# kcat/openal-soft

Measured on NVIDIA H100. Metric: voice-samples/s mixed (HRTF, bsinc24, 1024-frame updates), higher is better.
Workload: dtype f32

## Files before the change

### openal-soft_b200/csrc/mixer_kernels.cuh

```cuda
#pragma once
#include <cstdint>
#include <cuda_runtime.h>

#include "voice_structs.hpp"
#include "async_ptx.cuh"

namespace b200mix {

constexpr int kLine = 1024;
constexpr int kHrirLen = 128;
constexpr int kHist = 64;
constexpr int kEdge = 24;
constexpr int kPad = 48;
constexpr int kResBuf = kLine + 256 + kPad;
constexpr int kSrcSizeMax = kResBuf - kEdge;
constexpr int kAccumLen = kLine + kHrirLen;
constexpr float kSilence = 0.00001f;
constexpr float kEps = 1.1920929e-07f;

constexpr uint32_t kVfStatic = 1u<<2, kVfLooping = 1u<<3, kVfHrtf = 1u<<4;
constexpr uint32_t kVfFading = 1u<<8, kVfHaveBuffer = 1u<<9, kVfCoefDirty = 1u<<10;
constexpr uint32_t kUpNoBuffer = 1u<<11;
constexpr uint32_t kVfChannelMask = 0xffu<<16;

struct alignas(16) BufferRec {
    const void *data;
    uint32_t frames, type, channels, pad;
};

struct alignas(16) VoiceRec {
    uint32_t state;
    uint32_t flags;
    uint32_t buffer, resampler;
    int32_t  pos; uint32_t frac, step, loop_start;
    uint32_t loop_end; float bsinc_sf; uint32_t bsinc_m, bsinc_l;
    uint32_t bsinc_off, tgt_delay0, tgt_delay1; float tgt_gain;
    uint32_t old_delay0, old_delay1; float old_gain; uint32_t send_mask;
    uint32_t send_slot[kMaxSends]; uint32_t pad2[2];
    float prev[kPad];
    float hist[kHist];
};

struct VoiceResult { int32_t position; uint32_t position_frac, flags, buffers_done; };

struct alignas(16) FilterRec {
    float cur[2][5]; float tgt[2][5];
    float z[2][2];
    int32_t counter[2];
    uint32_t active;
    uint32_t pad[5];
};
static_assert(sizeof(FilterRec) == 128, "FilterRec layout");

struct MixParams {
    VoiceRec *voices; const BufferRec *buffers;
    float2 *hrtf_tgt; float2 *hrtf_old;
    float *dry_cur; float *dry_tgt;
    float *partial;
    VoiceResult *results;
    const float *bsinc_tab[3];
    const float *cubic_tab[2];
    uint32_t max_voices, frames, ir_pad, cd, num_sends;
    float *xscratch;
    uint32_t *sendinfo;
    const uint32_t *order;
    uint32_t num_order;
    FilterRec *filt;
    uint32_t filt_paths;
    const float *dline;
    uint4 *qhdr; const uint32_t *queue;
    uint32_t *claim;
};

constexpr uint32_t kMaxQueue = 32, kNoLoop = 0xffffffffu;

constexpr uint32_t kSiSend = 1u, kSiPlaying = 2u, kSiDeferred = 4u, kSiDirty = 8u, kSiDry = 16u,
    kSiHrtf = 32u;

__device__ __forceinline__ void group_sync(int id, int count)
{
    if(id == 1) asm volatile("bar.sync 1, %0;" :: "r"(count) : "memory");
    else asm volatile("bar.sync 2, %0;" :: "r"(count) : "memory");
}

__device__ __forceinline__ void prefetch_l2(const void *p)
{ asm volatile("prefetch.global.L2 [%0];" :: "l"(p)); }

__device__ __forceinline__ uint32_t sample_bytes(uint32_t type)
{ return type == 1u ? 2u : ((type == 0u || type >= 5u) ? 1u : (type == 4u ? 8u : 4u)); }

__device__ __forceinline__ void prefetch_span(const char *base, size_t bytes, size_t off,
    size_t len, int t, int gs)
{
    if(off >= bytes) return;
    if(off + len > bytes) len = bytes - off;
    const size_t first = off & ~size_t(127);
    for(size_t a = first + size_t(t)*128u;a < off + len;a += size_t(gs)*128u)
        prefetch_l2(base + a);
}

__device__ __forceinline__ float load_sample(const BufferRec &b, size_t idx)
{
    switch(b.type)
    {
    case 0: return (float(static_cast<const uint8_t*>(b.data)[idx]) - 128.0f) * (1.0f/128.0f);
    case 1: return float(static_cast<const int16_t*>(b.data)[idx]) * (1.0f/32768.0f);
    case 2: return float(static_cast<const int32_t*>(b.data)[idx]) * (1.0f/2147483648.0f);
    case 3: return static_cast<const float*>(b.data)[idx];
    case 4: return float(static_cast<const double*>(b.data)[idx]);
    }
    return 0.0f;
}

__device__ __forceinline__ void calc_buffer_size(uint32_t fracPos, uint32_t increment,
    uint32_t dstRemaining, uint32_t &dst, uint32_t &src)
{
    const uint32_t ext = increment <= 65536u;
    const uint64_t srcSize64 = ((uint64_t(dstRemaining - ext)*increment + fracPos) >> 16)
        + ext + kEdge;
    if(srcSize64 <= uint64_t(kSrcSizeMax)) { dst = dstRemaining; src = uint32_t(srcSize64); return; }
    const uint64_t dstSize64 = ((uint64_t(kSrcSizeMax - kEdge)<<16) - fracPos) / increment;
    if(dstSize64 < dstRemaining) { dst = uint32_t(dstSize64) & ~3u; src = kSrcSizeMax; return; }
    dst = dstRemaining; src = kSrcSizeMax;
}

__device__ __forceinline__ int32_t add_sat(int32_t a, int32_t b)
{
    long long r = (long long)a + b;
    r = r > 2147483647ll ? 2147483647ll : (r < -2147483648ll ? -2147483648ll : r);
    return int32_t(r);
}

__device__ __forceinline__ float to_float(uint8_t v) { return (float(v) - 128.0f) * (1.0f/128.0f); }
__device__ __forceinline__ float to_float(int16_t v) { return float(v) * (1.0f/32768.0f); }
__device__ __forceinline__ float to_float(int32_t v) { return float(v) * (1.0f/2147483648.0f); }
__device__ __forceinline__ float to_float(float v) { return v; }
__device__ __forceinline__ float to_float(double v) { return float(v); }
struct MulawByte { uint8_t v; };
struct AlawByte { uint8_t v; };
__device__ __forceinline__ float to_float(MulawByte b)
{
    const uint32_t u = (~uint32_t(b.v)) & 0xffu;
    const int s = int((((u & 0x0fu)<<3) + 0x84u) << ((u>>4)&7u)) - 0x84;
    return float((u & 0x80u) ? -s : s) * (1.0f/32768.0f);
}
__device__ __forceinline__ float to_float(AlawByte b)
{
    const uint32_t a = uint32_t(b.v) ^ 0x55u;
    const uint32_t e = (a>>4)&7u, m = a & 0x0fu;
    const int s = (e == 0u) ? int((m<<4) + 8u) : int(((m<<4) + 0x108u) << (e-1u));
    return float((a & 0x80u) ? s : -s) * (1.0f/32768.0f);
}

template<typename T> __device__ __forceinline__ T ld_raw(const T *p) { return __ldg(p); }
template<> __device__ __forceinline__ MulawByte ld_raw(const MulawByte *p)
{ return MulawByte{__ldg(reinterpret_cast<const uint8_t*>(p))}; }
template<> __device__ __forceinline__ AlawByte ld_raw(const AlawByte *p)
{ return AlawByte{__ldg(reinterpret_cast<const uint8_t*>(p))}; }

constexpr int kPackB = 688;
static_assert(kPackB >= (kResBuf + 8 + 1)/2 && kPackB + (kResBuf + 8 + 1)/2 <= kResBuf + 8 + 24
    && (kPackB % 32) == 16, "16-bit window copies must fit the float window's storage");

__device__ __forceinline__ float win_at(const float *win, bool packed, uint32_t k)
{
    if(!packed) return win[k];
    const uint16_t y = reinterpret_cast<const uint16_t*>(win)[k];
    return float(int(y) - 32768) * (1.0f/32768.0f);
}

struct FillArgs {
    float *dst; uint32_t count, uintPos, q0, firstRun, loopStart, loopSize, lastFrame, channels;
    bool looping, pastEnd, simpleWrap;
};

__device__ __forceinline__ void filter_clear(FilterRec &fr, int t)
{
    if(t < 10) fr.cur[t/5][t%5] = fr.tgt[t/5][t%5];
    else if(t < 14) fr.z[(t-10)>>1][(t-10)&1] = 0.0f;
    else if(t < 16) fr.counter[t-14] = 0;
}

template<typename T, int GS>
__device__ __forceinline__ void fill_window(const FillArgs &A, const T *__restrict__ src, int t)
{
    for(uint32_t k0 = t;k0 < A.count;k0 += 8u*GS)
    {
        T raw[8];
        #pragma unroll
        for(int u = 0;u < 8;++u)
        {
            uint32_t k = k0 + uint32_t(u)*GS;
            k = k < A.count ? k : A.count-1u;
            uint32_t q;
            if(!A.looping) q = min(A.uintPos + k, A.lastFrame);
            else if(k < A.firstRun) q = A.q0 + k;
            else if(A.simpleWrap) q = A.loopStart + (k - A.firstRun);
            else q = A.loopStart + (k - A.firstRun)%A.loopSize;
            raw[u] = ld_raw(src + size_t(q)*A.channels);
        }
        #pragma unroll
        for(int u = 0;u < 8;++u)
        {
            const uint32_t k = k0 + uint32_t(u)*GS;
            if(k < A.count) A.dst[k] = A.pastEnd ? 0.0f : to_float(raw[u]);
        }
    }
}

constexpr int kWinFloats = kResBuf + 8 + 24;
template<int CDR>
struct alignas(16) GroupSmem {
    static constexpr int kTabStride = kPad + 2;
    float win[kWinFloats];
    alignas(8) float tabF[32*kTabStride];
    alignas(8) float tabD[32*kTabStride];
    float x[CDR > 0 ? kLine : 1];
    float newGain[32];
    uint64_t tmaBar;
    uint32_t claimed;
};

template<int GS, int OPT, int FP>
struct alignas(16) FirSmem {
    static constexpr int kLLen = FP + OPT*GS;
    static constexpr int kOLen = FP + kHist + FP + 32;
    float2 lLR[kLLen];
    float2 oLR[kOLen];
    float x[kHist + kLine];
    float2 coefT[kHrirLen], coefO[kHrirLen];
};

__device__ __forceinline__ float2 fma2_rn(float2 a, float2 b, float2 c)
{ return make_float2(__fmaf_rn(a.x, b.x, c.x), __fmaf_rn(a.y, b.y, c.y)); }

template<int OPT, int FP>
__device__ __forceinline__ void fir_pass(float2 (&acc)[OPT], const float2 *__restrict__ in,
    const float2 *__restrict__ coef, int irpad, int t0)
{
    constexpr int JB = 8;
    constexpr int W = OPT + JB - 1;
    for(int jb = 0;jb < irpad;jb += 2*JB)
    {
        const float2 *p = in + FP + t0 - jb - (JB-1);
        float2 w[W];
        #pragma unroll
        for(int k = 0;k < W;++k) w[k] = p[k];
        #pragma unroll
        for(int jj = 0;jj < JB;++jj)
        {
            const float2 c = coef[jb+jj];
            #pragma unroll
            for(int r = 0;r < OPT;++r)
                acc[r] = fma2_rn(c, w[r - jj + (JB-1)], acc[r]);
        }
        if(jb + JB >= irpad) break;
        #pragma unroll
        for(int k = W-1;k >= JB;--k) w[k] = w[k-JB];
        #pragma unroll
        for(int k = 0;k < JB;++k) w[k] = p[k - JB];
        #pragma unroll
        for(int jj = 0;jj < JB;++jj)
        {
            const float2 c = coef[jb+JB+jj];
            #pragma unroll
            for(int r = 0;r < OPT;++r)
                acc[r] = fma2_rn(c, w[r - jj + (JB-1)], acc[r]);
        }
    }
}

__device__ __forceinline__ uint32_t claim_voice(const MixParams &P, uint32_t &slot, int t, int bar,
    int gs, uint32_t groups)
{
    group_sync(bar, gs);
    if(t == 0)
    {
        uint32_t oi = atomicAdd(P.claim, 1u);
        if(oi >= P.num_order && atomicAdd(P.claim + 1, 1u) == groups - 1u)
        {
            atomicExch(P.claim, 0u);
            atomicExch(P.claim + 1, 0u);
        }
        slot = oi;
    }
    group_sync(bar, gs);
    return slot;
}


__device__ __forceinline__ bool voice_early_out(const MixParams &P, VoiceRec &rec, uint32_t v,
    uint32_t vstate, uint4 h1, int t)
{
    if(vstate != 1u && vstate != 2u)
    {
        if(t == 0)
        {
            if(P.results) P.results[v] = VoiceResult{int32_t(h1.x), h1.y, 1u<<7, 0u};
            if(P.sendinfo) P.sendinfo[v] = 0u;
        }
        return true;
    }
    if(h1.z < 1u)
    {
        if(t == 0)
        {
            if(vstate == 2u) rec.state = 0u;
            if(P.sendinfo) P.sendinfo[v] = 0u;
            if(P.results)
                P.results[v] = VoiceResult{int32_t(h1.x), h1.y, (vstate == 2u) ? (1u<<7) : 1u, 0u};
        }
        return true;
    }
    return false;
}

template<int GS>
__device__ __forceinline__ void build_phase_table(const MixParams &P, float *tabF, float *tabD,
    uint32_t resampler, uint32_t increment, uint4 h2, uint4 h3, int t,
    uint32_t &m, uint32_t &tapOff, uint32_t &ms)
{
    m = 0; tapOff = 0; ms = 5;
    if(resampler >= 4u)
    {
        m = h2.z;
        tapOff = kEdge - h2.w;
        const float *tab = P.bsinc_tab[(resampler-4u)>>1] + h3.x;
        const bool full = (increment > 65536u) && (resampler & 1u);
        const float sf = __uint_as_float(h2.y);
        const uint32_t rowLen = 2u*m;
        const float *tab2 = tab + 64u*m;
        ms = m + 1u;
        for(uint32_t c = t;c < rowLen;c += GS)
        {
            float *dstc = (c < m) ? (tabF + c) : (tabD + (c - m));
            #pragma unroll 1
            for(uint32_t p0 = 0;p0 < 32u;p0 += 8u)
            {
                float a[8], b[8];
                #pragma unroll
                for(int u = 0;u < 8;++u)
                {
                    a[u] = __ldg(tab + (p0+u)*rowLen + c);
                    b[u] = full ? __ldg(tab2 + (p0+u)*rowLen + c) : 0.0f;
                }
                #pragma unroll
                for(int u = 0;u < 8;++u)
                    dstc[(p0+u)*ms] = full ? fmaf(sf, b[u], a[u]) : a[u];
            }
        }
    }
    else if(resampler >= 2u)
    {
        m = 4; tapOff = kEdge - 1; ms = 5;
        const float *tab = P.cubic_tab[resampler-2u];
        for(uint32_t e = t;e < 128u;e += GS)
        {
            const uint32_t pi = e>>2, j = e&3u;
            tabF[pi*ms + j] = tab[pi*8u + j];
            tabD[pi*ms + j] = tab[pi*8u + 4u + j];
        }
    }
}

template<int GS>
__device__ __forceinline__ void prefetch_next_voices(const MixParams &P, uint32_t oi, uint32_t groups,
    int t)
{
    const uint32_t o2 = oi + 2u*groups, o1 = oi + groups;
    const uint32_t v2 = o2 < P.num_order ? P.order[o2] : 0xffffffffu;
    const uint32_t v1 = o1 < P.num_order ? P.order[o1] : 0xffffffffu;
    if(v2 < P.max_voices && t < 5)
        prefetch_l2(reinterpret_cast<const char*>(&P.voices[v2]) + t*128);
    if(v1 < P.max_voices)
    {
        const VoiceRec &nx = P.voices[v1];
        if((nx.state == 1u || nx.state == 2u) && (nx.flags & kVfHaveBuffer) && nx.step >= 1u)
        {
            const BufferRec nb = P.buffers[nx.buffer];
            const size_t fb = size_t(sample_bytes(nb.type))*nb.channels;
            const size_t bytes = size_t(nb.frames)*fb;
            const uint32_t p0 = nx.pos < 0 ? 0u : uint32_t(nx.pos);
            const size_t need = size_t((uint64_t(P.frames)*nx.step + nx.frac) >> 16) + kPad;
            const char *base = static_cast<const char*>(nb.data);
            prefetch_span(base, bytes, size_t(p0)*fb, need*fb, t, GS);
            if((nx.flags & kVfLooping) && p0 + need > nx.loop_end && nx.loop_end > p0)
                prefetch_span(base, bytes, size_t(nx.loop_start)*fb,
                    (p0 + need - nx.loop_end)*fb, t, GS);
        }
    }
}

template<int GS>
__device__ __forceinline__ void hold_end_sample(float *srcBuffer, uint32_t srcn, int t, int bar)
{
    const uint32_t avail = srcn < uint32_t(kEdge) ? srcn : uint32_t(kEdge);
    const uint32_t tofill = srcn > uint32_t(kEdge) ? srcn : uint32_t(kEdge);
    uint32_t best = 0;
    for(uint32_t i = 1;i < avail;++i)
        if(fabsf(srcBuffer[i]) < fabsf(srcBuffer[best])) best = i;
    const float held = srcBuffer[best];
    group_sync(bar, GS);
    for(uint32_t k = best+1+t;k < tofill;k += GS) srcBuffer[k] = held;
}

template<int GS>
__device__ __forceinline__ void pack_span16(float *win, const unsigned char *raw, uint32_t lead,
    uint32_t srcDelay, uint32_t count, int t, int bar)
{
    constexpr int NW = (kResBuf + 8 + 1)/2;
    constexpr int PER = (NW + GS - 1)/GS;
    static_assert((GS/32)*(32*PER - 1) >= NW + 1, "the warps' runs must cover every word");
    const uint32_t lane = uint32_t(t) & 31u;
    const uint32_t w0 = uint32_t(t >> 5)*(32u*PER - 1u) + lane;
    const uint32_t lo = uint32_t(kEdge) + srcDelay;
    const uint32_t nw = (min(lo + count + 8u, uint32_t(kResBuf + 8)) + 1u)/2u;
    const uint32_t off = lo - lead;
    const uint32_t *rw = reinterpret_cast<const uint32_t*>(raw) - int((off + 1u) >> 1);
    const uint32_t sh = (off & 1u)*16u;
    uint32_t wa[PER];
    #pragma unroll
    for(int u = 0;u < PER;++u)
    {
        const uint32_t w = w0 + uint32_t(u)*32u;
        wa[u] = (w <= nw && 2u*w + 1u >= lo) ? rw[w] : 0u;
    }
    #pragma unroll
    for(int u = 0;u < PER;++u)
    {
        const uint32_t w = w0 + uint32_t(u)*32u;
        uint32_t r1 = __shfl_sync(0xffffffffu, (u + 1 < PER && lane == 0u) ? wa[u + 1 < PER ? u + 1 : u] : wa[u],
            (lane + 1u) & 31u);
        if(u + 1 == PER && lane == 31u && w <= nw && 2u*w + 3u >= lo) r1 = rw[w + 1u];
        uint32_t a = __funnelshift_r(wa[u], r1, sh) ^ 0x80008000u;
        const int d = int(lo) - int(2u*w);
        const uint32_t m = (d >= 1 ? 0x0000ffffu : 0u) | (d >= 2 ? 0xffff0000u : 0u);
        a = (a & ~m) | (0x80008000u & m);
        if(u == 0 && w < uint32_t(kEdge/2))
            a = uint32_t(uint16_t(__float2int_rn(win[2u*w]*32768.0f) + 32768))
                | (uint32_t(uint16_t(__float2int_rn(win[2u*w + 1u]*32768.0f) + 32768)) << 16);
        wa[u] = a;
    }
    group_sync(bar, GS);
    uint32_t *pa = reinterpret_cast<uint32_t*>(win);
    uint32_t *pb = pa + kPackB;
    #pragma unroll
    for(int u = 0;u < PER;++u)
    {
        const uint32_t w = w0 + uint32_t(u)*32u;
        const uint32_t next = __shfl_sync(0xffffffffu, (u + 1 < PER && lane == 0u) ? wa[u + 1 < PER ? u + 1 : u] : wa[u],
            (lane + 1u) & 31u);
        if(w < nw)
        {
            if(u > 0 || lane > 0u || t < 32) pa[w] = wa[u];
            if(u + 1 < PER || lane < 31u) pb[w] = __funnelshift_r(wa[u], next, 16u);
        }
    }
}

template<int GS>
__device__ __forceinline__ bool stage_span_tma(float *win, uint64_t *tmaBar, uint32_t &tmaPhase,
    const BufferRec &buf, uint32_t flags, bool isQueue, bool looping, uint32_t loopStart,
    uint32_t loopEnd, uint32_t uintPos, uint32_t srcDelay, uint32_t count, bool pack, bool &packed,
    int t, int bar)
{
    if(isQueue || buf.type != 1u || buf.channels != 1u || ((flags >> 16) & 0xffu) != 0u || count == 0u)
        return false;
    const uint32_t loopSize = looping ? (loopEnd - loopStart) : 1u;
    const uint32_t q0 = !looping ? uintPos : ((uintPos < loopEnd) ? uintPos
        : ((uintPos-loopStart)%loopSize + loopStart));
    const uint32_t run1 = looping ? min(count, loopEnd - q0) : count;
    const uint32_t run2 = count - run1;
    const bool fits = looping ? (run2 <= loopSize && loopEnd <= buf.frames)
                              : (uintPos + count <= buf.frames);
    if(!fits) return false;
    const int16_t *base = static_cast<const int16_t*>(buf.data);
    const uintptr_t a1 = reinterpret_cast<uintptr_t>(base + q0);
    const uintptr_t a2 = reinterpret_cast<uintptr_t>(base + loopStart);
    const uint32_t lead1 = uint32_t(a1 & 15u) >> 1, lead2 = uint32_t(a2 & 15u) >> 1;
    const uint32_t bytes1 = ((run1 + lead1)*2u + 15u) & ~15u;
    const uint32_t bytes2 = run2 ? (((run2 + lead2)*2u + 15u) & ~15u) : 0u;
    constexpr uint32_t kWinBytes = uint32_t(kWinFloats*sizeof(float));
    unsigned char *wbytes = reinterpret_cast<unsigned char*>(win);
    unsigned char *raw2 = wbytes + kWinBytes - bytes2;
    unsigned char *raw1 = raw2 - bytes1;
    if(t == 0)
    {
        fence_proxy_async_smem();
        mbar_expect_tx(tmaBar, bytes1 + bytes2);
        bulk_g2s(raw1, reinterpret_cast<const void*>(a1 & ~uintptr_t(15)), bytes1, tmaBar);
        if(run2)
            bulk_g2s(raw2, reinterpret_cast<const void*>(a2 & ~uintptr_t(15)), bytes2, tmaBar);
    }
    mbar_wait(tmaBar, tmaPhase);
    tmaPhase ^= 1u;
    if(pack && !run2)
    {
        pack_span16<GS>(win, raw1, lead1, srcDelay, count, t, bar);
        packed = true;
        return true;
    }
    float *dst = win + kEdge + srcDelay;
    const int16_t *r1 = reinterpret_cast<const int16_t*>(raw1) + lead1;
    const int16_t *r2 = reinterpret_cast<const int16_t*>(raw2) + lead2;
    constexpr int PERW = (kSrcSizeMax + GS - 1)/GS;
    float v[PERW];
    #pragma unroll
    for(int u = 0;u < PERW;++u)
    {
        const uint32_t k = uint32_t(t) + uint32_t(u)*GS;
        int16_t x = 0;
        if(k < count) x = k < run1 ? r1[k] : r2[k - run1];
        v[u] = to_float(x);
    }
    group_sync(bar, GS);
    #pragma unroll
    for(int u = 0;u < PERW;++u)
    {
        const uint32_t k = uint32_t(t) + uint32_t(u)*GS;
        if(k < count) dst[k] = v[u];
    }
    return true;
}

template<int GS>
__device__ __forceinline__ bool gather_span(const MixParams &P, const BufferRec &buf, uint32_t flags,
    bool isQueue, uint4 qh, const uint32_t *qitems, bool looping, uint32_t loopStart, uint32_t loopEnd,
    uint32_t uintPos, uint32_t count, float *dst, int t, int bar)
{
    uint32_t done = 0, item = qh.x ? qh.y : kNoLoop, qpos = uintPos;
    bool more = true, winInt = true;
    while(more)
    {
// ... 252 lines not shown
    {
        const float cg = counter ? cur[c] : tgt[c];
        const float tg = playing ? tgt[c] : 0.0f;
        const float step = (tg - cg)*delta;
        const bool fade = fabsf(step) > kEps;
        const bool early = fade && fadeLen < counter;
        const float flat = (!early && fabsf(tg) > kSilence) ? tg : 0.0f;
        const uint32_t start = fade ? fadeLen : 0u;
        #pragma unroll
        for(int r = 0;r < SPT;++r)
        {
            const uint32_t i = t + r*GS;
            float gsel = 0.0f;
            if(i < n)
                gsel = (fade && i < fadeLen) ? (cg + step*float(i)) : (i >= start ? flat : 0.0f);
            const float x = xs[i < n ? i : 0];
            if(c < uint32_t(CDR))
            {
                #pragma unroll
                for(int cc = 0;cc < CDR;++cc)
                    if(cc == int(c)) accD[cc][r] = __fmaf_rn(x, gsel, accD[cc][r]);
            }
        }
        if(t == 0)
            newGain[c] = early ? (cg + step*float(fadeLen)) : tg;
    }
}

__device__ __forceinline__ void store_dry_gains(float *cur, const float *newGain, uint32_t cd, int t)
{
    if(t == 0)
        for(uint32_t c = 0;c < cd;++c) cur[c] = newGain[c];
}

__device__ __forceinline__ void write_back_voice(const MixParams &P, VoiceRec &rec, uint32_t v,
    uint4 h1, uint32_t flags, uint32_t vstate, uint32_t increment, bool haveBuffer, bool isQueue,
    uint4 qh, const uint32_t *qitems, bool looping, uint32_t loopStart, uint32_t loopEnd,
    uint32_t bufFrames)
{
    uint32_t newFlags = (flags | kVfFading) & ~kVfCoefDirty;
    uint32_t newState = vstate;
    uint32_t buffersDone = 0u;
    int32_t pos = int32_t(h1.x); uint32_t frac = h1.y;
    if(vstate == 2u) newState = 0u;
    else
    {
        frac += increment*P.frames;
        const uint32_t done = frac >> 16;
        pos = add_sat(pos, int32_t(done));
        frac &= 0xffffu;
        if(haveBuffer && pos > 0 && isQueue)
        {
            uint32_t item = qh.x ? qh.y : kNoLoop;
            while(item != kNoLoop)
            {
                const uint32_t len = P.buffers[qitems[item]].frames;
                if(len > uint32_t(pos)) break;
                pos -= int32_t(len);
                ++buffersDone;
                item = (item + 1u < qh.x) ? item + 1u : qh.z;
            }
            if(item == kNoLoop) { newFlags &= ~kVfHaveBuffer; newState = 2u; }
            else if(item != qh.y) P.qhdr[v].y = item;
        }
        else if(haveBuffer && pos > 0)
        {
            if(looping)
            {
                uint32_t up = uint32_t(pos);
                if(up >= loopEnd)
                    pos = int32_t((up-loopStart)%(loopEnd-loopStart) + loopStart);
            }
            else if(uint32_t(pos) >= bufFrames)
            {
                newFlags &= ~kVfHaveBuffer;
                newState = 2u;
            }
        }
        rec.pos = pos; rec.frac = frac;
    }
    rec.flags = newFlags;
    rec.state = newState;
    if(P.results)
        P.results[v] = VoiceResult{pos, frac,
            newState == 1u ? 1u : (newState == 2u ? 2u : (1u<<7)), buffersDone};
}

template<int GS, int GROUPS, int CDR>
__device__ __forceinline__ void store_partial_row(const float (&accD)[CDR][kLine/GS], unsigned char *smem,
    float *partial, int g, int t)
{
    constexpr int SPT = kLine / GS;
    const size_t row = blockIdx.x;
    __syncthreads();
    float *stage = reinterpret_cast<float*>(smem);
    float *pd = partial + row*(size_t(CDR)*kLine);
    if(GROUPS == 1)
    {
        #pragma unroll
        for(int c = 0;c < CDR;++c)
            #pragma unroll
            for(int r = 0;r < SPT;++r)
                pd[c*kLine + t + r*GS] = accD[c][r];
    }
    else
    {
        for(int gg = 0;gg < GROUPS;++gg)
        {
            if(g == gg)
            {
                #pragma unroll
                for(int c = 0;c < CDR;++c)
                    #pragma unroll
                    for(int r = 0;r < SPT;++r)
                    {
                        float *dst = stage + c*kLine + t + r*GS;
                        if(gg == 0) *dst = accD[c][r]; else *dst += accD[c][r];
                    }
            }
            __syncthreads();
        }
        for(int o = threadIdx.x;o < CDR*kLine;o += GS*GROUPS) pd[o] = stage[o];
    }
}

constexpr int kMixGS = 64, kMixGroups = 2;

template<int GS, int GROUPS, int CDR>
__global__ void __launch_bounds__(GS*GROUPS, GS*GROUPS != 128 ? 1 : (CDR == 0 ? 5 : 3))
k_mix_voices(const MixParams P)
{
    using Smem = GroupSmem<CDR>;
    static_assert(CDR == 0 || sizeof(Smem)*GROUPS >= size_t(CDR)*kLine*sizeof(float),
        "the partial row is staged in the groups' storage");
    extern __shared__ __align__(16) unsigned char smem_raw[];
    const int g = threadIdx.x / GS;
    const int t = threadIdx.x % GS;
    Smem &S = reinterpret_cast<Smem*>(smem_raw)[g];
    const int bar = 1 + g;
    constexpr int SPT = kLine / GS;

    float accD[CDR > 0 ? CDR : 1][SPT];
    #pragma unroll
    for(int c = 0;c < (CDR > 0 ? CDR : 1);++c)
        #pragma unroll
        for(int r = 0;r < SPT;++r) accD[c][r] = 0.0f;

    const uint32_t n = P.frames;
    if(t == 0) { mbar_init(&S.tmaBar, 1u); mbar_fence_init(); }
    uint32_t tmaPhase = 0u;
    group_sync(bar, GS);

    const uint32_t groups = gridDim.x*GROUPS;
    for(uint32_t oi = CDR > 0 ? blockIdx.x*GROUPS + g : claim_voice(P, S.claimed, t, bar, GS, groups);
        oi < P.num_order;
        oi = CDR > 0 ? oi + groups : claim_voice(P, S.claimed, t, bar, GS, groups))
    {
        const uint32_t v = P.order[oi];
        VoiceRec &rec = P.voices[v];
        const uint4 *hp = reinterpret_cast<const uint4*>(&rec);
        const uint4 h0 = hp[0], h1 = hp[1], h2 = hp[2], h3 = hp[3];
        const uint32_t vstate = h0.x;
        if(voice_early_out(P, rec, v, vstate, h1, t)) continue;
        const uint32_t increment = h1.z;
        const uint32_t flags = h0.y;
        const bool haveBuffer = (flags & kVfHaveBuffer) != 0;
        const BufferRec buf = P.buffers[haveBuffer ? h0.z : 0u];
        const uint32_t loopStart = h1.w, loopEnd = h2.x;
        int32_t intPos = int32_t(h1.x);
        uint32_t fracPos = h1.y;
        bool looping = (flags & kVfLooping) != 0;
        if((flags & kVfStatic) && looping && haveBuffer && intPos >= 0
            && uint32_t(intPos) >= loopEnd)
            looping = false;
        const uint32_t resampler = h0.w;
        const bool isQueue = !(flags & kVfStatic) && P.qhdr != nullptr;
        const uint4 qh = isQueue ? P.qhdr[v] : make_uint4(0u, 0u, kNoLoop, 0u);
        const uint32_t *qitems = P.queue + size_t(v)*kMaxQueue;
        const bool isHrtf = CDR == 0 && P.ir_pad != 0u && (flags & kVfHrtf);
        const bool dirty = (flags & kVfCoefDirty) != 0;
        FilterRec *dfilt = P.filt ? P.filt + size_t(v)*P.filt_paths : nullptr;
        const bool defer = dfilt && dfilt->active;
        const bool playing = vstate == 1u;

        for(int k = t;k < kPad;k += GS) S.win[k] = rec.prev[k];
        uint32_t m, tapOff, ms;
        build_phase_table<GS>(P, S.tabF, S.tabD, resampler, increment, h2, h3, t, m, tapOff, ms);
        float *xs = CDR > 0 ? S.x : P.xscratch + size_t(v)*kLine;
        if(CDR == 0) prefetch_next_voices<GS>(P, oi, groups, t);

        for(uint32_t loaded = 0;loaded < n;)
        {
            uint32_t dstn, srcn;
            calc_buffer_size(fracPos, increment, n-loaded, dstn, srcn);
            uint32_t srcDelay = 0;
            bool silent = false;
            bool packedWin = false;
            if(dstn == 0u) { dstn = n - loaded; silent = true; }
            if(intPos < 0)
            {
                srcDelay = uint32_t(-intPos);
                if(srcDelay >= srcn) silent = true;
            }
            group_sync(bar, GS);
            if(silent)
            {
                for(uint32_t k = t;k < dstn;k += GS) xs[loaded+k] = 0.0f;
                for(uint32_t k = t;k < srcn;k += GS) S.win[kEdge+k] = 0.0f;
            }
            else
            {
                float *srcBuffer = S.win + kEdge;
                bool winInt = false;
                const bool pack = resampler >= 4u && !(increment == 65536u && fracPos == 0u);
                if(!haveBuffer) hold_end_sample<GS>(srcBuffer, srcn, t, bar);
                else
                {
                    const uint32_t uintPos = intPos < 0 ? 0u : uint32_t(intPos);
                    const uint32_t count = srcn - srcDelay;
                    for(uint32_t k = t;k < srcDelay;k += GS) srcBuffer[k] = 0.0f;
                    winInt = stage_span_tma<GS>(S.win, &S.tmaBar, tmaPhase, buf, flags, isQueue, looping,
                            loopStart, loopEnd, uintPos, srcDelay, count, pack, packedWin, t, bar)
                        || gather_span<GS>(P, buf, flags, isQueue, qh, qitems, looping, loopStart, loopEnd,
                            uintPos, count, srcBuffer + srcDelay, t, bar);
                }
                group_sync(bar, GS);

                if(pack && winInt && !packedWin)
                {
                    pack_window16<GS>(S.win, srcn, t, bar);
                    packedWin = true;
                }
                resample_chunk<GS>(S.win, S.tabF, S.tabD, xs, loaded, dstn, increment, fracPos,
                    resampler, m, tapOff, ms, packedWin, t);
            }
            advance_chunk<GS>(S.win, rec.prev, packedWin, silent, playing, n, loaded, dstn, increment,
                fracPos, intPos, t, bar);
        }
        group_sync(bar, GS);

        const uint32_t counter = (flags & kVfFading) ? (n < 64u ? n : 64u) : 0u;
        if(P.sendinfo)
            park_voice<GS, CDR>(P, xs, v, rec.send_mask, defer, isHrtf, playing, dirty, counter, t);
        if(dfilt && !defer) filter_clear(*dfilt, t);
        if constexpr(CDR > 0)
            if(!defer)
                mix_dry<GS, CDR>(accD, xs, S.newGain, P.dry_cur + size_t(v)*P.cd, P.dry_tgt + size_t(v)*P.cd,
                    P.cd, n, counter, playing, t);
        if(t == 0)
            write_back_voice(P, rec, v, h1, flags, vstate, increment, haveBuffer, isQueue, qh, qitems,
                looping, loopStart, loopEnd, buf.frames);
        group_sync(bar, GS);
        if(CDR > 0 && !defer) store_dry_gains(P.dry_cur + size_t(v)*P.cd, S.newGain, P.cd, t);
        group_sync(bar, GS);
    }

    if constexpr(CDR > 0) store_partial_row<GS, GROUPS, CDR>(accD, smem_raw, P.partial, g, t);
}

template<int GROUPS, int CDR>
union DeferredSmem {
    struct { float x[kLine]; float newGain[32]; } group[GROUPS];
    float stage[CDR*kLine];
};

template<int GS, int GROUPS, int CDR>
__global__ void __launch_bounds__(GS*GROUPS)
k_mix_deferred(const MixParams P)
{
    extern __shared__ __align__(16) unsigned char smem_raw[];
    const int g = threadIdx.x / GS;
    const int t = threadIdx.x % GS;
    auto &S = reinterpret_cast<DeferredSmem<GROUPS, CDR>*>(smem_raw)->group[g];
    const int bar = 1 + g;
    constexpr int SPT = kLine / GS;

    float accD[CDR][SPT];
    #pragma unroll
    for(int c = 0;c < CDR;++c)
        #pragma unroll
        for(int r = 0;r < SPT;++r) accD[c][r] = 0.0f;

    const uint32_t n = P.frames;
    const uint32_t groups = gridDim.x*GROUPS;
    for(uint32_t oi = blockIdx.x*GROUPS + g;oi < P.num_order;oi += groups)
    {
        const uint32_t v = P.order[oi];
        const uint32_t info = P.sendinfo[v];
        if(!(info & kSiDeferred)) continue;
        const float *fl = P.dline + size_t(v)*kLine;
        for(uint32_t k = t;k < n;k += GS) S.x[k] = fl[k];
        group_sync(bar, GS);
        mix_dry<GS, CDR>(accD, S.x, S.newGain, P.dry_cur + size_t(v)*P.cd, P.dry_tgt + size_t(v)*P.cd,
            P.cd, n, (info >> 8) & 0xffu, (info & kSiPlaying) != 0, t);
        group_sync(bar, GS);
        store_dry_gains(P.dry_cur + size_t(v)*P.cd, S.newGain, P.cd, t);
    }

    store_partial_row<GS, GROUPS, CDR>(accD, smem_raw, P.partial, g, t);
}

constexpr int kFirGS = 64, kFirGroups = 2, kFirCtasPerSm = 4;

template<int OPT, int FP>
__global__ void __launch_bounds__(kFirGS*kFirGroups, kFirCtasPerSm)
k_hrtf_fir(const MixParams P)
{
    constexpr int GS = kFirGS, GROUPS = kFirGroups;
    using Smem = FirSmem<GS, OPT, FP>;
    extern __shared__ __align__(16) unsigned char smem_raw[];
    const int g = threadIdx.x / GS;
    const int t = threadIdx.x % GS;
    Smem &S = reinterpret_cast<Smem*>(smem_raw)[g];
    const int bar = 1 + g;
    const int t0 = OPT*t;
    const uint32_t n = P.frames;

    float2 acc[OPT];
    #pragma unroll
    for(int r = 0;r < OPT;++r) acc[r] = make_float2(0.0f, 0.0f);

    const uint32_t stride = gridDim.x*GROUPS;
    for(uint32_t oi = blockIdx.x*GROUPS + g;oi < P.num_order;oi += stride)
    {
        const uint32_t v = P.order[oi];
        const uint32_t info = P.sendinfo[v];
        if(!(info & kSiHrtf)) continue;
        VoiceRec &rec = P.voices[v];
        const uint4 *hp = reinterpret_cast<const uint4*>(&rec);
        const uint4 h3 = hp[3], h4 = hp[4];
        const bool playing = (info & kSiPlaying) != 0;
        const bool dirty = (info & kSiDirty) != 0;
        const uint32_t counter = (info >> 8) & 0xffu;

        const float *line = ((info & kSiDeferred) ? P.dline : P.xscratch) + size_t(v)*kLine;
        for(int k = t;k < kHist;k += GS) S.x[k] = rec.hist[k];
        for(uint32_t k = t;k < n;k += GS) S.x[kHist + k] = line[k];
        const float2 *ct = P.hrtf_tgt + size_t(v)*P.ir_pad;
        const float2 *co = P.hrtf_old + size_t(v)*P.ir_pad;
        for(int k = t;k < int(P.ir_pad);k += GS)
        {
            const float2 c = ct[k];
            S.coefT[k] = c;
            S.coefO[k] = dirty ? co[k] : c;
        }
        group_sync(bar, GS);


        if(playing)
            for(int k = t;k < kHist;k += GS) rec.hist[k] = S.x[n + k];
        uint32_t oD0 = h4.x, oD1 = h4.y;
        float oGain = __uint_as_float(h4.z);
        const uint32_t tD0 = h3.y, tD1 = h3.z;
        const float tgtGain = __uint_as_float(h3.w);
        if(!counter) { oD0 = tD0; oD1 = tD1; oGain = tgtGain; }
        const bool sameFilter = !counter || (!dirty && oD0 == tD0 && oD1 == tD1);
        const float targetGain = tgtGain * (playing ? 1.0f : 0.0f);
        const uint32_t fademix = counter;
        float blendNewStep = 0.0f, oldStep = 0.0f;
        bool oldOn = false, newOn = false;
        float gainA = oGain;
        if(fademix)
        {
            const float gain = targetGain;
            blendNewStep = gain / float(fademix);
            oldStep = oGain / float(fademix);
            oldOn = oGain > kSilence;
            newOn = blendNewStep*float(fademix) > kSilence;
            gainA = gain;
        }
        const uint32_t todo = n - fademix;
        const float step2 = todo ? (targetGain - gainA) / float(todo) : 0.0f;

        const float *hs = S.x;
        for(int i = t;i < Smem::kLLen;i += GS)
        {
            const int s = i - FP;
            float l = 0.0f, r = 0.0f;
            if(s >= 0 && s < int(n))
            {
                float gnew;
                if(uint32_t(s) < fademix)
                    gnew = (newOn && s >= 1) ? blendNewStep*float(s) : 0.0f;
                else
                    gnew = gainA + step2*float(uint32_t(s) - fademix);
                l = hs[kHist - tD0 + s] * gnew;
                r = hs[kHist - tD1 + s] * gnew;
                if(sameFilter && oldOn && uint32_t(s) < fademix)
                {
                    const float gold = oldStep*float(fademix - uint32_t(s));
                    l += hs[kHist - oD0 + s] * gold;
                    r += hs[kHist - oD1 + s] * gold;
                }
            }
            S.lLR[i] = make_float2(l, r);
        }
        const bool oldPass = !sameFilter && oldOn;
        if(oldPass)
            for(int i = t;i < Smem::kOLen;i += GS)
            {
                const int s = i - FP;
                float l = 0.0f, r = 0.0f;
                if(s >= 0 && uint32_t(s) < fademix)
                {
                    const float gold = oldStep*float(fademix - uint32_t(s));
                    l = hs[kHist - oD0 + s] * gold;
                    r = hs[kHist - oD1 + s] * gold;
                }
                S.oLR[i] = make_float2(l, r);
            }
        group_sync(bar, GS);

        {
            const uint32_t o2 = oi + 2u*stride, o1 = oi + stride;
            const uint32_t v2 = o2 < P.num_order ? P.order[o2] : 0xffffffffu;
            const uint32_t v1 = o1 < P.num_order ? P.order[o1] : 0xffffffffu;
            if(v2 < P.max_voices)
            {
                if(t < 5) prefetch_l2(reinterpret_cast<const char*>(&P.voices[v2]) + t*128);
                else if(t < 5 + int((P.ir_pad*8u + 127u)/128u))
                    prefetch_l2(reinterpret_cast<const char*>(P.hrtf_tgt + size_t(v2)*P.ir_pad) + (t-5)*128);
            }
            if(v1 < P.max_voices && t < int(kLine*sizeof(float)/128u))
            {
                const float *nl = ((P.sendinfo[v1] & kSiDeferred) ? P.dline : P.xscratch) + size_t(v1)*kLine;
                prefetch_l2(reinterpret_cast<const char*>(nl) + t*128);
            }
        }

        const int irpad = int(P.ir_pad);
        fir_pass<OPT, FP>(acc, S.lLR, S.coefT, irpad, t0);
        if(oldPass && t0 < int(kHist) + irpad)
            fir_pass<OPT, FP>(acc, S.oLR, S.coefO, irpad, t0);
        if(t == 0)
        {
            rec.old_delay0 = tD0; rec.old_delay1 = tD1;
            rec.old_gain = targetGain;
        }
        group_sync(bar, GS);
    }

    const size_t row = blockIdx.x;
    __syncthreads();
    float *stage = reinterpret_cast<float*>(smem_raw);
    for(int gg = 0;gg < GROUPS;++gg)
    {
        if(g == gg)
        {
            #pragma unroll
            for(int r = 0;r < OPT;++r)
            {
                const int o = t0 + r;
                if(o < kAccumLen)
                {
                    if(gg == 0) { stage[o] = acc[r].x; stage[kAccumLen + o] = acc[r].y; }
                    else { stage[o] += acc[r].x; stage[kAccumLen + o] += acc[r].y; }
                }
            }
            if(gg == 0 && GS*OPT < kAccumLen)
                for(int o = GS*OPT + t;o < kAccumLen;o += GS) { stage[o] = 0.0f; stage[kAccumLen + o] = 0.0f; }
        }
        __syncthreads();
    }
    float *pl = P.partial + row*(2*kAccumLen);
    for(int o = threadIdx.x;o < 2*kAccumLen;o += GS*GROUPS) pl[o] = stage[o];
}


constexpr int kReduceCols = 8, kReduceSegs = 128;
__global__ void __launch_bounds__(1024)
k_reduce_rows(const float *__restrict__ partial, uint32_t rows, uint32_t len,
    float *__restrict__ out, int accumulate)
{
    __shared__ float4 sm[kReduceSegs][kReduceCols];
    const uint32_t col = threadIdx.x & (kReduceCols-1), seg = threadIdx.x / kReduceCols;
    const uint32_t e4 = blockIdx.x*kReduceCols + col;
    float4 s = make_float4(0.f, 0.f, 0.f, 0.f);
    if(e4*4u < len)
    {
        const uint32_t per = (rows + kReduceSegs - 1u)/kReduceSegs;
        const uint32_t r0 = seg*per, r1 = (r0 + per < rows) ? r0 + per : rows;
        const float4 *p = reinterpret_cast<const float4*>(partial) + e4;
        const size_t stride4 = len/4u;
        uint32_t r = r0;
        for(;r + 4u <= r1;r += 4u)
        {
            const float4 a = __ldg(p + size_t(r)*stride4), b = __ldg(p + size_t(r+1)*stride4);
            const float4 c = __ldg(p + size_t(r+2)*stride4), d = __ldg(p + size_t(r+3)*stride4);
            s.x += a.x; s.y += a.y; s.z += a.z; s.w += a.w;
            s.x += b.x; s.y += b.y; s.z += b.z; s.w += b.w;
            s.x += c.x; s.y += c.y; s.z += c.z; s.w += c.w;
            s.x += d.x; s.y += d.y; s.z += d.z; s.w += d.w;
        }
        for(;r < r1;++r)
        {
            const float4 a = __ldg(p + size_t(r)*stride4);
            s.x += a.x; s.y += a.y; s.z += a.z; s.w += a.w;
        }
    }
    sm[seg][col] = s;
    __syncthreads();
    #pragma unroll
    for(uint32_t width = kReduceSegs/4u;width >= 1u;width /= 4u)
    {
        float4 tot = make_float4(0.f, 0.f, 0.f, 0.f);
        const bool on = seg < width;
        if(on)
        {
            tot = sm[seg*4u][col];
            #pragma unroll
            for(uint32_t k = 1;k < 4u;++k)
            {
                const float4 a = sm[seg*4u + k][col];
                tot.x += a.x; tot.y += a.y; tot.z += a.z; tot.w += a.w;
            }
        }
        __syncthreads();
        if(on) sm[seg][col] = tot;
        __syncthreads();
        if(width == 2u) break;
    }
    if(seg == 0 && e4*4u < len)
    {
        float4 tot = sm[0][col];
        const float4 b = sm[1][col];
        tot.x += b.x; tot.y += b.y; tot.z += b.z; tot.w += b.w;
        float4 *o = reinterpret_cast<float4*>(out) + e4;
        if(accumulate)
        {
            const float4 a = *o;
            tot.x += a.x; tot.y += a.y; tot.z += a.z; tot.w += a.w;
        }
        *o = tot;
    }
}

__global__ void __launch_bounds__(256)
k_reduce_few(const float *__restrict__ partial, uint32_t rows, uint32_t len,
    float *__restrict__ out, int accumulate)
{
    const uint32_t e4 = blockIdx.x*blockDim.x + threadIdx.x;
    if(e4*4u >= len) return;
    const float4 *p = reinterpret_cast<const float4*>(partial) + e4;
    const size_t stride4 = len/4u;
    float4 v[16];
    #pragma unroll
    for(uint32_t r = 0;r < 16u;++r)
        v[r] = r < rows ? __ldg(p + size_t(r)*stride4) : make_float4(0.f, 0.f, 0.f, 0.f);
    float4 g[4];
    #pragma unroll
    for(uint32_t j = 0;j < 4u;++j)
    {
        float4 t = v[4u*j];
        #pragma unroll
        for(uint32_t k = 1;k < 4u;++k)
        { t.x += v[4u*j+k].x; t.y += v[4u*j+k].y; t.z += v[4u*j+k].z; t.w += v[4u*j+k].w; }
        g[j] = t;
    }
    float4 tot = g[0];
    #pragma unroll
    for(uint32_t j = 1;j < 4u;++j) { tot.x += g[j].x; tot.y += g[j].y; tot.z += g[j].z; tot.w += g[j].w; }
    float4 *o = reinterpret_cast<float4*>(out) + e4;
    if(accumulate)
    {
        const float4 a = *o;
        tot.x += a.x; tot.y += a.y; tot.z += a.z; tot.w += a.w;
    }
    *o = tot;
}

struct ApplyParams {
    VoiceRec *voices; const VoiceUpdate *updates;
    const float *coeffs; const float *dry; const float *send;
    float2 *hrtf_tgt; float2 *hrtf_old; float *dry_cur, *dry_tgt, *send_cur, *send_tgt;
    uint32_t ir, ir_pad, cd, cw, num_sends;
    FilterRec *filt; uint32_t filt_paths;
    const float4 *dirs;
    const float2 *st_fields;
    const uint2 *st_elevs;
    const float2 *st_coeffs;
    const uint8_t *st_delays;
    uint32_t st_num_fields, st_ir;
    uint4 *qhdr;
};

struct HrirBlend { uint32_t idx[4]; float w[4]; float passthru; uint32_t delay[2]; };

__device__ __forceinline__ void hrir_index(uint32_t count, float v, bool elev, uint32_t &idx, float &blend)
{
    const float inv_pi = 0.318309886183790671538f;
    if(elev)
    {
        v = __fmul_rn(__fadd_rn(__fmul_rn(inv_pi, v), 0.5f), float(count-1u));
        const uint32_t i = v > 0.0f ? uint32_t(v) : 0u;
        idx = min(i, count-1u); blend = __fsub_rn(v, float(i));
    }
    else
    {
        v = __fmul_rn(__fadd_rn(__fmul_rn(inv_pi*0.5f, v), 1.0f), float(count));
        const uint32_t i = v > 0.0f ? uint32_t(v) : 0u;
        idx = i % count; blend = __fsub_rn(v, float(i));
    }
}

__device__ __forceinline__ void hrir_blend(const ApplyParams &A, const float4 dir, HrirBlend &B)
{
    const float inv_pi = 0.318309886183790671538f;
    const float elevation = dir.x, azimuth = dir.y, distance = dir.z, spread = dir.w;
    const float dirfact = __fsub_rn(1.0f, __fmul_rn(inv_pi/2.0f, spread));
    uint32_t ebase = 0, fi = 0;
    for(;fi + 1u < A.st_num_fields;++fi)
    {
        if(distance >= A.st_fields[fi].x) break;
        ebase += __float_as_uint(A.st_fields[fi].y);
    }
    const uint32_t evCount = __float_as_uint(A.st_fields[fi].y);
    uint32_t e0i; float e0b;
    hrir_index(evCount, elevation, true, e0i, e0b);
    const uint32_t e1i = min(e0i + 1u, evCount - 1u);
    const uint2 el0 = A.st_elevs[ebase + e0i], el1 = A.st_elevs[ebase + e1i];
    uint32_t a0i, a1i; float a0b, a1b;
    hrir_index(el0.x, azimuth, false, a0i, a0b);
    hrir_index(el1.x, azimuth, false, a1i, a1b);
    B.idx[0] = el0.y + a0i; B.idx[1] = el0.y + ((a0i + 1u) % el0.x);
    B.idx[2] = el1.y + a1i; B.idx[3] = el1.y + ((a1i + 1u) % el1.x);
    const float ne = __fsub_rn(1.0f, e0b);
    B.w[0] = __fmul_rn(__fmul_rn(ne, __fsub_rn(1.0f, a0b)), dirfact);
    B.w[1] = __fmul_rn(__fmul_rn(ne, a0b), dirfact);
    B.w[2] = __fmul_rn(__fmul_rn(e0b, __fsub_rn(1.0f, a1b)), dirfact);
    B.w[3] = __fmul_rn(__fmul_rn(e0b, a1b), dirfact);
    #pragma unroll
    for(int ear = 0;ear < 2;++ear)
    {
        float dsum = __fmul_rn(float(A.st_delays[B.idx[0]*2u + ear]), B.w[0]);
        dsum = __fadd_rn(dsum, __fmul_rn(float(A.st_delays[B.idx[1]*2u + ear]), B.w[1]));
        dsum = __fadd_rn(dsum, __fmul_rn(float(A.st_delays[B.idx[2]*2u + ear]), B.w[2]));
        dsum = __fadd_rn(dsum, __fmul_rn(float(A.st_delays[B.idx[3]*2u + ear]), B.w[3]));
        B.delay[ear] = uint32_t(__float2int_rn(__fmul_rn(dsum, 0.25f)));
    }
    B.passthru = __fmul_rn(0.70710678118654752440f, __fsub_rn(1.0f, dirfact));
}

__device__ __forceinline__ void filter_reset_word(FilterRec *fr, int k)
{
    uint32_t *w = reinterpret_cast<uint32_t*>(fr);
    uint32_t val = 0u;
    if(k == 0 || k == 5 || k == 10 || k == 15) val = __float_as_uint(1.0f);
    else if(k == 24 || k == 25) val = 0xffffffffu;
    w[k] = val;
}

struct QueueSet { uint32_t voice, count, loop; uint32_t items[kMaxQueue]; };
__global__ void k_set_queue(VoiceRec *voices, uint4 *qhdr, uint32_t *queue, const QueueSet Q)
{
    const uint32_t t = threadIdx.x;
    if(t < Q.count) queue[size_t(Q.voice)*kMaxQueue + t] = Q.items[t];
    if(t == 0)
    {
        qhdr[Q.voice] = make_uint4(Q.count, 0u, Q.loop, 0u);
        uint32_t fl = voices[Q.voice].flags;
        fl = Q.count ? (fl | kVfHaveBuffer) : (fl & ~kVfHaveBuffer);
        voices[Q.voice].flags = fl;
    }
}

__global__ void k_filter_init(FilterRec *filt, size_t count)
{
    const size_t i = size_t(blockIdx.x)*blockDim.x + threadIdx.x;
    if(i < count*32u) filter_reset_word(filt + (i >> 5), int(i & 31u));
}

__global__ void k_apply_filter_updates(FilterRec *filt, uint32_t paths, const FilterUpdate *upd,
    uint32_t n)
{
    const uint32_t i = blockIdx.x*blockDim.x + threadIdx.x;
    if(i >= n*2u) return;
    const FilterUpdate &u = upd[i >> 1];
    const int f = int(i & 1u);
    FilterRec &fr = filt[size_t(u.voice)*paths + u.path];
    const float *nt = f ? u.hp : u.lp;
    bool diff = false;
    #pragma unroll
    for(int k = 0;k < 5;++k)
    {
        diff |= !(fabsf(nt[k] - fr.tgt[f][k]) <= 0.015625f);
        fr.tgt[f][k] = nt[k];
    }
    const int c = fr.counter[f];
    if(!diff)
    {
        if(c <= 0)
        {
            fr.counter[f] = 0;
            #pragma unroll
            for(int k = 0;k < 5;++k) fr.cur[f][k] = nt[k];
        }
    }
    else if(c >= 0) fr.counter[f] = 8*32;
    else
    {
        fr.counter[f] = 0;
        #pragma unroll
        for(int k = 0;k < 5;++k) fr.cur[f][k] = nt[k];
    }
    if(f == 0) fr.active = u.active ? 1u : 0u;
}

__global__ void __launch_bounds__(64) k_apply_updates(const ApplyParams A)
{
    const uint32_t u = blockIdx.x;
    const VoiceUpdate up = A.updates[u];
    VoiceRec &rec = A.voices[up.voice];
    const int t = threadIdx.x;
    const bool reset = (up.flags & (1u<<5)) != 0;
    const uint32_t oldFlags = reset ? 0u : rec.flags;
    const bool wasDirty = (oldFlags & kVfCoefDirty) != 0;
    __syncthreads();
    if(reset)
    {
        for(int k = t;k < kPad;k += 64) rec.prev[k] = 0.0f;
        for(int k = t;k < kHist;k += 64) rec.hist[k] = 0.0f;
        if(A.dry_cur) for(uint32_t c = t;c < A.cd;c += 64) A.dry_cur[size_t(up.voice)*A.cd + c] = 0.0f;
        if(A.send_cur)
            for(uint32_t c = t;c < A.num_sends*A.cw;c += 64)
                A.send_cur[size_t(up.voice)*A.num_sends*A.cw + c] = 0.0f;
        if(A.filt)
            for(uint32_t k = t;k < A.filt_paths*32u;k += 64)
                filter_reset_word(A.filt + size_t(up.voice)*A.filt_paths + (k >> 5), int(k & 31u));
    }
    __shared__ HrirBlend sB;
    const bool fromDirs = A.dirs != nullptr && up.has_coeffs && A.hrtf_tgt;
    if(fromDirs)
    {
        if(t == 0) hrir_blend(A, A.dirs[u], sB);
        __syncthreads();
    }
    if(up.has_coeffs && A.hrtf_tgt)
    {
        float2 *tg = A.hrtf_tgt + size_t(up.voice)*A.ir_pad;
        float2 *ol = A.hrtf_old + size_t(up.voice)*A.ir_pad;
        const float *src = fromDirs ? nullptr : A.coeffs + size_t(u)*A.ir*2;
        for(uint32_t k = t;k < A.ir_pad;k += 64)
// ... 873 lines not shown
```

Before: 29.66 billion.

## Double-buffer HRTF FIR voice inputs with bulk async copies and mbarriers

Replaces the per-voice cooperative loads of history, input line and HRIR coefficients in the HRTF FIR kernel with bulk global-to-shared async copies into a two-stage buffer. Thread 0 issues the next voice's copies while the current voice is processed, and an mbarrier wait replaces the load-then-sync step. The explicit L2 prefetches are dropped. The gain-application loop is split into a fade segment and a steady segment, and zero padding of lLR is hoisted out of the voice loop. This costs extra shared memory per group, which may reduce occupancy, and adds mbarrier parity bookkeeping.

```diff
diff --git a/openal-soft_b200/csrc/mixer_kernels.cuh b/openal-soft_b200/csrc/mixer_kernels.cuh
--- a/openal-soft_b200/csrc/mixer_kernels.cuh
+++ b/openal-soft_b200/csrc/mixer_kernels.cuh
@@ -1,4 +1,5 @@
 #pragma once
+#include <cstddef>
 #include <cstdint>
 #include <cuda_runtime.h>
 
@@ -221,14 +222,21 @@
     uint32_t claimed;
 };
 
+struct alignas(16) FirStage {
+    float x[kHist + kLine];
+    float2 coefT[kHrirLen], coefO[kHrirLen];
+};
+static_assert(offsetof(VoiceRec, hist) % 16 == 0 && sizeof(VoiceRec) % 16 == 0,
+    "VoiceRec::hist is a bulk-copy source: 16-byte aligned");
+
 template<int GS, int OPT, int FP>
 struct alignas(16) FirSmem {
     static constexpr int kLLen = FP + OPT*GS;
     static constexpr int kOLen = FP + kHist + FP + 32;
     float2 lLR[kLLen];
     float2 oLR[kOLen];
-    float x[kHist + kLine];
-    float2 coefT[kHrirLen], coefO[kHrirLen];
+    FirStage st[2];
+    uint64_t bar[2];
 };
 
 __device__ __forceinline__ float2 fma2_rn(float2 a, float2 b, float2 c)
@@ -1087,6 +1095,32 @@
 
 constexpr int kFirGS = 64, kFirGroups = 2, kFirCtasPerSm = 4;
 
+__device__ __forceinline__ uint32_t next_hrtf_voice(const MixParams &P, uint32_t oi, uint32_t stride,
+    uint32_t &v, uint32_t &info)
+{
+    for(;oi < P.num_order;oi += stride)
+    {
+        v = P.order[oi];
+        info = P.sendinfo[v];
+        if(info & kSiHrtf) break;
+    }
+    return oi;
+}
+
+__device__ __forceinline__ void fir_stage_issue(const MixParams &P, FirStage &B, uint64_t *bar,
+    uint32_t v, uint32_t info, uint32_t n)
+{
+    const uint32_t lineBytes = (n & ~3u)*4u, irBytes = P.ir_pad*8u;
+    const bool dirty = (info & kSiDirty) != 0;
+    const float *line = ((info & kSiDeferred) ? P.dline : P.xscratch) + size_t(v)*kLine;
+    fence_proxy_async_smem();
+    mbar_expect_tx(bar, kHist*4u + lineBytes + (dirty ? 2u : 1u)*irBytes);
+    bulk_g2s(B.x, P.voices[v].hist, kHist*4u, bar);
+    if(lineBytes) bulk_g2s(B.x + kHist, line, lineBytes, bar);
+    bulk_g2s(B.coefT, P.hrtf_tgt + size_t(v)*P.ir_pad, irBytes, bar);
+    if(dirty) bulk_g2s(B.coefO, P.hrtf_old + size_t(v)*P.ir_pad, irBytes, bar);
+}
+
 template<int OPT, int FP>
 __global__ void __launch_bounds__(kFirGS*kFirGroups, kFirCtasPerSm)
 k_hrtf_fir(const MixParams P)
@@ -1105,35 +1139,39 @@
     #pragma unroll
     for(int r = 0;r < OPT;++r) acc[r] = make_float2(0.0f, 0.0f);
 
+    for(int i = t;i < FP;i += GS) S.lLR[i] = make_float2(0.0f, 0.0f);
+    for(int i = FP + int(n) + t;i < Smem::kLLen;i += GS) S.lLR[i] = make_float2(0.0f, 0.0f);
+    if(t == 0) { mbar_init(&S.bar[0], 1u); mbar_init(&S.bar[1], 1u); mbar_fence_init(); }
+    group_sync(bar, GS);
+
     const uint32_t stride = gridDim.x*GROUPS;
-    for(uint32_t oi = blockIdx.x*GROUPS + g;oi < P.num_order;oi += stride)
-    {
-        const uint32_t v = P.order[oi];
-        const uint32_t info = P.sendinfo[v];
-        if(!(info & kSiHrtf)) continue;
+    uint32_t v = 0u, info = 0u;
+    uint32_t oi = next_hrtf_voice(P, blockIdx.x*GROUPS + g, stride, v, info);
+    if(t == 0 && oi < P.num_order) fir_stage_issue(P, S.st[0], &S.bar[0], v, info, n);
+    uint32_t parity = 0u;
+    for(int b = 0;oi < P.num_order;b ^= 1)
+    {
         VoiceRec &rec = P.voices[v];
         const uint4 *hp = reinterpret_cast<const uint4*>(&rec);
         const uint4 h3 = hp[3], h4 = hp[4];
+
+        uint32_t vN = 0u, infoN = 0u;
+        const uint32_t oiN = next_hrtf_voice(P, oi + stride, stride, vN, infoN);
+        if(t == 0 && oiN < P.num_order) fir_stage_issue(P, S.st[b^1], &S.bar[b^1], vN, infoN, n);
+
+        FirStage &B = S.st[b];
         const bool playing = (info & kSiPlaying) != 0;
         const bool dirty = (info & kSiDirty) != 0;
         const uint32_t counter = (info >> 8) & 0xffu;
 
         const float *line = ((info & kSiDeferred) ? P.dline : P.xscratch) + size_t(v)*kLine;
-        for(int k = t;k < kHist;k += GS) S.x[k] = rec.hist[k];
-        for(uint32_t k = t;k < n;k += GS) S.x[kHist + k] = line[k];
-        const float2 *ct = P.hrtf_tgt + size_t(v)*P.ir_pad;
-        const float2 *co = P.hrtf_old + size_t(v)*P.ir_pad;
-        for(int k = t;k < int(P.ir_pad);k += GS)
-        {
-            const float2 c = ct[k];
-            S.coefT[k] = c;
-            S.coefO[k] = dirty ? co[k] : c;
-        }
-        group_sync(bar, GS);
-
+        for(uint32_t k = (n & ~3u) + t;k < n;k += GS) B.x[kHist + k] = line[k];
+        mbar_wait(&S.bar[b], (parity >> b) & 1u);
+        parity ^= 1u << b;
+        if(n & 3u) group_sync(bar, GS);
 
         if(playing)
-            for(int k = t;k < kHist;k += GS) rec.hist[k] = S.x[n + k];
+            for(int k = t;k < kHist;k += GS) rec.hist[k] = B.x[n + k];
         uint32_t oD0 = h4.x, oD1 = h4.y;
         float oGain = __uint_as_float(h4.z);
         const uint32_t tD0 = h3.y, tD1 = h3.z;
@@ -1157,28 +1195,26 @@
         const uint32_t todo = n - fademix;
         const float step2 = todo ? (targetGain - gainA) / float(todo) : 0.0f;
 
-        const float *hs = S.x;
-        for(int i = t;i < Smem::kLLen;i += GS)
-        {
-            const int s = i - FP;
-            float l = 0.0f, r = 0.0f;
-            if(s >= 0 && s < int(n))
-            {
-                float gnew;
-                if(uint32_t(s) < fademix)
-                    gnew = (newOn && s >= 1) ? blendNewStep*float(s) : 0.0f;
-                else
-                    gnew = gainA + step2*float(uint32_t(s) - fademix);
-                l = hs[kHist - tD0 + s] * gnew;
-                r = hs[kHist - tD1 + s] * gnew;
-                if(sameFilter && oldOn && uint32_t(s) < fademix)
-                {
-                    const float gold = oldStep*float(fademix - uint32_t(s));
-                    l += hs[kHist - oD0 + s] * gold;
-                    r += hs[kHist - oD1 + s] * gold;
-                }
-            }
-            S.lLR[i] = make_float2(l, r);
+        const float *hs = B.x;
+        float2 *in = S.lLR + FP;
+        for(uint32_t s = t;s < fademix;s += GS)
+        {
+            const float gnew = (newOn && s >= 1u) ? blendNewStep*float(s) : 0.0f;
+            float l = hs[kHist - tD0 + s] * gnew;
+            float r = hs[kHist - tD1 + s] * gnew;
+            if(sameFilter && oldOn)
+            {
+                const float gold = oldStep*float(fademix - s);
+                l += hs[kHist - oD0 + s] * gold;
+                r += hs[kHist - oD1 + s] * gold;
+            }
+            in[s] = make_float2(l, r);
+        }
+        const float *xl = hs + kHist - tD0, *xr = hs + kHist - tD1;
+        for(uint32_t s = fademix + t;s < n;s += GS)
+        {
+            const float gnew = gainA + step2*float(s - fademix);
+            in[s] = make_float2(xl[s] * gnew, xr[s] * gnew);
         }
         const bool oldPass = !sameFilter && oldOn;
         if(oldPass)
@@ -1196,33 +1232,17 @@
             }
         group_sync(bar, GS);
 
-        {
-            const uint32_t o2 = oi + 2u*stride, o1 = oi + stride;
-            const uint32_t v2 = o2 < P.num_order ? P.order[o2] : 0xffffffffu;
-            const uint32_t v1 = o1 < P.num_order ? P.order[o1] : 0xffffffffu;
-            if(v2 < P.max_voices)
-            {
-                if(t < 5) prefetch_l2(reinterpret_cast<const char*>(&P.voices[v2]) + t*128);
-                else if(t < 5 + int((P.ir_pad*8u + 127u)/128u))
-                    prefetch_l2(reinterpret_cast<const char*>(P.hrtf_tgt + size_t(v2)*P.ir_pad) + (t-5)*128);
-            }
-            if(v1 < P.max_voices && t < int(kLine*sizeof(float)/128u))
-            {
-                const float *nl = ((P.sendinfo[v1] & kSiDeferred) ? P.dline : P.xscratch) + size_t(v1)*kLine;
-                prefetch_l2(reinterpret_cast<const char*>(nl) + t*128);
-            }
-        }
-
         const int irpad = int(P.ir_pad);
-        fir_pass<OPT, FP>(acc, S.lLR, S.coefT, irpad, t0);
+        fir_pass<OPT, FP>(acc, S.lLR, B.coefT, irpad, t0);
         if(oldPass && t0 < int(kHist) + irpad)
-            fir_pass<OPT, FP>(acc, S.oLR, S.coefO, irpad, t0);
+            fir_pass<OPT, FP>(acc, S.oLR, dirty ? B.coefO : B.coefT, irpad, t0);
         if(t == 0)
         {
             rec.old_delay0 = tD0; rec.old_delay1 = tD1;
             rec.old_gain = targetGain;
         }
         group_sync(bar, GS);
+        oi = oiN; v = vN; info = infoN;
     }
 
     const size_t row = blockIdx.x;
```

Result: faster. 30.97 billion (median of 6 runs) (+4.4%).
